# GATB/bcalm

Measured on AMD Instinct MI355X. Metric: distinct k-mers/s reads->unitigs k=31, higher is better.
Workload: dtype u64; 1 GPU; BASELINE config 3: synthetic 100000000 x 150 bp reads per GPU, k=31, abundance-min 2, 1% substitutions, 30x coverage; multi_gpu=single GPU, minimizer_size=16, log2_partitions=22

## Files before the change

bcalm_amd/csrc/host_ctx.h:

```cpp
#pragma once

namespace {

thread_local std::string g_err;
int fail(int code, const char* fmt, ...) {
    char buf[512];
    va_list ap; va_start(ap, fmt); vsnprintf(buf, sizeof buf, fmt, ap); va_end(ap);
    g_err = buf;
    return code;
}
#define HIPCK(call)                                                                                   \
    do {                                                                                              \
        hipError_t e_ = (call);                                                                       \
        if (e_ != hipSuccess)                                                                         \
            return fail(e_ == hipErrorOutOfMemory ? CDBG_E_NOMEM : CDBG_E_NODEVICE, "%s failed: %s (%s:%d)", \
                        #call, hipGetErrorString(e_), __FILE__, __LINE__);                            \
    } while (0)
#define CK(expr) do { int rc_ = (expr); if (rc_ != CDBG_OK) return rc_; } while (0)

struct DevPool {
    static constexpr size_t MIN_BYTES = 1u << 20;
    struct Block { void* p; size_t bytes; };
    std::mutex mu; std::vector<Block> blocks[64]; size_t held[64] = {}; size_t limit_[64] = {};
    static int device() { int d = 0; if (hipGetDevice(&d) != hipSuccess || d < 0 || d >= 64) d = 0; return d; }
// ... 230 lines not shown
    std::vector<uint64_t> run_off, run_start, run_place; std::vector<uint32_t> run_len; bool runs_ready = false;
    DBuf<uint32_t> comp, comp_first; DBuf<uint64_t> comp_unitigs, comp_bases, comp_kmers, comp_kc; bool comp_ready = false; uint64_t comp_info[5] = { 0, 0, 0, 0, 0 };
    DBuf<uint32_t> color_planes, color_ustart; uint32_t color_n = 0; uint64_t color_words = 0; bool color_opened = false; DBuf<uint64_t> color_out;
    DBuf<uint64_t> cl_run_off, cl_runs, cl_kmers; DBuf<uint32_t> cl_offset, cl_len, cl_cls, cl_ncol, cl_bits; bool cl_ready = false; uint64_t color_info[4] = { 0, 0, 0, 0 };
    DBuf<uint64_t> cq_seg_off, cq_seg_start, cq_seg_place; DBuf<uint32_t> cq_seg_len, cq_seg_cls, cq_found, cq_ncol, cq_bits;
    bool cq_ready = false; uint64_t cq_n = 0, cq_segs = 0;
    DBuf<uint4> rank_a, rank_b; DBuf<uint32_t> rank_flag;
    DBuf<uint4> walk_rec; DBuf<uint32_t> walk_heads, walk_hlen; DBuf<uint64_t> walk_hoff; bool walk_off = false;
    cdbg_transport tr{}; bool have_tr = false; uint64_t comm_bytes = 0;
    bool tr_ordered = false;
    bool force_multi = false;
#ifndef CDBG_HOSTSIM
    RcclComm* rccl = nullptr;
#endif
    DBuf<uint32_t> xcnt; DBuf<uint64_t> xoff, xbase, xrecs;
    uint64_t piece_lo = 0, piece_hi = 0;
    bool xchg_done = false;
    DBuf<uint8_t> xg[5], xsend;
    DBuf<uint8_t> dg_dest, dg_dense, dg_packed, dg_rpacked, dg_rdense; DBuf<uint64_t> dg_pos, dg_cnt, dg_wire_s, dg_wire_r, dg_meta_s, dg_meta_r, dg_boff, dg_uoff, dg_rboff, dg_rkc, dg_aoff, dg_raoff;
    DBuf<uint2> dg_pairs, dg_pair_s, dg_pair_r, dg_rs, dg_rr; DBuf<uint32_t> dg_qs, dg_qsrc, dg_qr, dg_lens, dg_alen, dg_rn, dg_rlens, dg_ab_s, dg_ab_r, dg_rab; DBuf<uint4> dg_rst;
};

namespace {

int stream_scan_dispatch(cdbg_ctx* c);
int ingest_init(cdbg_ctx* c) {
    if (c->pin[0]) return CDBG_OK;
    if (const char* e = c->knobs.get("CDBG_STAGE_BYTES")) c->stage_bytes = std::min<uint64_t>(cdbg_ctx::STAGE_BYTES, std::max<uint64_t>(64, strtoull(e, nullptr, 10)));
    HIPCK(hipStreamCreate(&c->copy_stream));
    for (int i = 0; i < 2; ++i) {
        if (hipHostMalloc((void**)&c->pin[i], cdbg_ctx::STAGE_BYTES) != hipSuccess) return fail(CDBG_E_NOMEM, "pinned staging buffer (%llu bytes)", (unsigned long long)cdbg_ctx::STAGE_BYTES);
        HIPCK(hipEventCreate(&c->pin_ev[i]));
    }
    return CDBG_OK;
}
void ingest_release(cdbg_ctx* c) {
    for (int i = 0; i < 2; ++i) {
        if (c->pin[i]) { (void)hipHostFree(c->pin[i]); (void)hipEventDestroy(c->pin_ev[i]); c->pin[i] = nullptr; }
    }
    for (auto& sg : c->stages) if (sg.p) { (void)hipHostFree(sg.p); (void)hipEventDestroy(sg.ev); }
    c->stages.clear();
    if (c->copy_stream) { (void)hipStreamDestroy(c->copy_stream); c->copy_stream = hipStream_t{}; }
}
int ingest_reserve(cdbg_ctx* c, uint64_t need) {
    while (c->prewarm_reads.load(std::memory_order_acquire)) std::this_thread::sleep_for(std::chrono::microseconds(200));
    if (c->reads.p && c->reads.cap >= need) return CDBG_OK;
    uint64_t cap = std::max<uint64_t>(c->reads.cap * 2, 256ull << 20);
    if (c->expect_bytes) cap = std::max<uint64_t>(cap, c->expect_bytes + c->expect_bytes / 64 + (8ull << 20));
    while (cap < need) cap *= 2;
    if (c->ss_on) HIPCK(hipStreamSynchronize(c->stream));
    DBuf<uint8_t> bigger;
    CK(bigger.alloc(cap, false));
    HIPCK(hipStreamSynchronize(c->copy_stream));
    if (c->n_dev) HIPCK(hipMemcpy(bigger.p, c->reads.p, c->n_dev, hipMemcpyDeviceToDevice));
    c->reads.swap(bigger);
    return CDBG_OK;
}
int ingest_flush(cdbg_ctx* c) {
    if (!c->pin_fill) return CDBG_OK;
    CK(ingest_reserve(c, c->n_dev + c->pin_fill));
    const int b = c->pin_cur;
    HIPCK(hipMemcpyAsync(c->reads.p + c->n_dev, c->pin[b], c->pin_fill, hipMemcpyHostToDevice, c->copy_stream));
    HIPCK(hipEventRecord(c->pin_ev[b], c->copy_stream));
    c->pin_busy[b] = true;
    c->n_dev += c->pin_fill; c->pin_fill = 0;
    c->pin_cur = b ^ 1;
    if (c->pin_busy[b ^ 1]) { HIPCK(hipEventSynchronize(c->pin_ev[b ^ 1])); c->pin_busy[b ^ 1] = false; }
    if (c->expect_bytes && c->prm.world_size == 1 && !c->force_multi) CK(stream_scan_dispatch(c));
    return CDBG_OK;
}
int ingest_append(cdbg_ctx* c, const char* src, uint64_t n) {
    CK(ingest_init(c));
    while (n) {
        const uint64_t room = c->stage_bytes - c->pin_fill, take = std::min(room, n);
        memcpy(c->pin[c->pin_cur] + c->pin_fill, src, take);
        c->pin_fill += take; src += take; n -= take;
        if (c->pin_fill == c->stage_bytes) CK(ingest_flush(c));
    }
    return CDBG_OK;
}
int stage_acquire(cdbg_ctx* c, char** buf, uint64_t* cap) {
    CK(ingest_init(c));
    for (;;) {
        int oldest = -1;
        for (int i = 0; i < (int)c->stages.size(); ++i) {
            cdbg_ctx::Stage& sg = c->stages[i];
            if (sg.state == 2 && hipEventQuery(sg.ev) == hipSuccess) sg.state = 0;
            if (sg.state == 0) { sg.state = 1; *buf = (char*)sg.p; *cap = c->stage_bytes; return CDBG_OK; }
            if (sg.state == 2 && oldest < 0) oldest = i;
        }
        if ((int)c->stages.size() >= 32 && oldest >= 0) { HIPCK(hipEventSynchronize(c->stages[oldest].ev)); continue; }
        if ((int)c->stages.size() < cdbg_ctx::MAX_STAGES) {
            cdbg_ctx::Stage sg;
            if (hipHostMalloc((void**)&sg.p, cdbg_ctx::STAGE_BYTES) != hipSuccess) return fail(CDBG_E_NOMEM, "pinned staging buffer (%llu bytes)", (unsigned long long)cdbg_ctx::STAGE_BYTES);
            if (hipEventCreate(&sg.ev) != hipSuccess) { (void)hipHostFree(sg.p); return fail(CDBG_E_NODEVICE, "hipEventCreate failed (staging buffer)"); }
            sg.state = 1; c->stages.push_back(sg);
            *buf = (char*)sg.p; *cap = c->stage_bytes; return CDBG_OK;
        }
        if (oldest < 0) return fail(CDBG_E_STATE, "cdbg_stage_acquire: all %d staging buffers are held by the caller", cdbg_ctx::MAX_STAGES);
        HIPCK(hipEventSynchronize(c->stages[oldest].ev));
    }
}
int ingest_flush(cdbg_ctx* c);
int stage_commit(cdbg_ctx* c, char* buf, uint64_t n) {
    cdbg_ctx::Stage* sg = nullptr;
    for (auto& x : c->stages) if ((char*)x.p == buf) sg = &x;
    if (!sg || sg->state != 1) return fail(CDBG_E_PARAM, "cdbg_stage_commit: not a buffer handed out by cdbg_stage_acquire");
    if (n > c->stage_bytes) return fail(CDBG_E_PARAM, "cdbg_stage_commit: %llu bytes in a buffer of %llu", (unsigned long long)n, (unsigned long long)c->stage_bytes);
    if (n && base_valid((uint8_t)buf[n - 1])) {
        if (n == c->stage_bytes) return fail(CDBG_E_PARAM, "cdbg_stage_commit: a full buffer must end with a separator");
        buf[n++] = '\n';
    }
    if (!n) { sg->state = 0; return CDBG_OK; }
    CK(ingest_flush(c));
    CK(ingest_reserve(c, c->n_dev + n));
    HIPCK(hipMemcpyAsync(c->reads.p + c->n_dev, buf, n, hipMemcpyHostToDevice, c->copy_stream));
    HIPCK(hipEventRecord(sg->ev, c->copy_stream));
    sg->state = 2;
    c->n_dev += n;
    if (c->expect_bytes && c->prm.world_size == 1 && !c->force_multi) CK(stream_scan_dispatch(c));
    return CDBG_OK;
}
int upload_pending(cdbg_ctx* c) {
    if (c->reads_final) return CDBG_OK;
    if (c->n_dev == 0 && c->pin_fill == 0) {
        if (c->prm.world_size > 1 || c->force_multi) {
            CK(c->reads.alloc(512, false));
            HIPCK(hipMemset(c->reads.p, '\n', 512));
            c->nbytes = 0; c->nbytes_padded = 256; c->reads_final = true;
        }
        return CDBG_OK;
    }
    CK(ingest_flush(c));
    const uint64_t n = c->n_dev;
    const uint64_t np = ((n + 15) / 16) * 16 + 256;
    CK(ingest_reserve(c, np));
    HIPCK(hipStreamSynchronize(c->copy_stream));
    HIPCK(hipMemset(c->reads.p + n, '\n', np - n));
    c->nbytes = n; c->nbytes_padded = np; c->reads_final = true;
    ingest_release(c);
    return CDBG_OK;
}

int read_u64(const uint64_t* dptr, uint64_t* out, size_t n = 1) {
    HIPCK(hipMemcpy(out, dptr, n * sizeof(uint64_t), hipMemcpyDeviceToHost));
    return CDBG_OK;
}
int read_u32(const uint32_t* dptr, uint32_t* out, size_t n = 1) {
    HIPCK(hipMemcpy(out, dptr, n * sizeof(uint32_t), hipMemcpyDeviceToHost));
    return CDBG_OK;
}
int check_device_error(cdbg_ctx* c, const char* where) {
    uint32_t e = 0; CK(read_u32(c->derr.p, &e));
    if (e) return fail(CDBG_E_INTERNAL, "%s: device reported error %u (1 solid overflow, 2 scratch sizing, 3 piece overflow, 4 unitig overflow, 5 glue log overflow, 9 junction-ownership flag of a k-mer wrong [simulator build only])", where, e);
    HIPCK(hipGetLastError());
    return CDBG_OK;
}
struct HostMarks {
    bool on = enabled(); double t0 = now();
    static bool enabled() { static const bool e = getenv("CDBG_HOST_MARKS") != nullptr; return e; }
    static double now() { timespec ts; clock_gettime(CLOCK_MONOTONIC, &ts); return ts.tv_sec * 1e3 + ts.tv_nsec * 1e-6; }
    void mark(const char* what) { if (!on) return; (void)hipDeviceSynchronize(); const double t = now(); fprintf(stderr, "[host] %-28s %8.2f ms\n", what, t - t0); t0 = t; }
};
struct Timer {
    hipEvent_t a{}, b{}; hipStream_t s{};
    int start(hipStream_t st) { s = st; HIPCK(hipEventCreate(&a)); HIPCK(hipEventCreate(&b)); HIPCK(hipEventRecord(a, s)); return CDBG_OK; }
    int stop(float* ms) { HIPCK(hipEventRecord(b, s)); HIPCK(hipEventSynchronize(b)); HIPCK(hipEventElapsedTime(ms, a, b)); (void)hipEventDestroy(a); (void)hipEventDestroy(b); return CDBG_OK; }
};

void configure(cdbg_ctx* c, uint64_t total_bytes) {
    const int W = c->W;
    const int ts = W == 1 ? TS_COUNT_1 : W == 2 ? TS_COUNT_2 : TS_COUNT_4;
#ifndef CDBG_OCC_NUM
#define CDBG_OCC_NUM 3
#define CDBG_OCC_DEN 2
#endif
    const bool sifted = W >= 3 && c->prm.abundance_min >= 2;
    const uint64_t target_occ = W >= 3 ? (uint64_t)ts * (sifted ? 12 : 6) / 10 : (uint64_t)ts * CDBG_OCC_NUM / CDBG_OCC_DEN;
    int log_np = c->log_np_override >= 0 ? c->log_np_override : c->prm.log2_partitions;
    if (log_np < 0) {
        log_np = 0;
        while (log_np < 24 && ((uint64_t)1 << log_np) * target_occ < total_bytes) ++log_np;
    }
    if (log_np < c->rank_bits) log_np = c->rank_bits;
    if (log_np > 26) log_np = 26;
    int m = c->prm.minimizer_size;
    if (m <= 0) m = std::min(16, std::max(6, (log_np + 10) / 2 + 1));
    m = std::max(1, std::min(m, std::min(16, c->k - 1)));
    c->log_np = log_np; c->m = m;
    c->n_local_parts = ((uint64_t)1 << log_np) >> c->rank_bits;
    c->st.minimizer_size = m; c->st.log2_partitions = log_np; c->st.kmer_words = W;
}

int exscan_u32(cdbg_ctx* c, const uint32_t* counts, uint64_t* off, uint64_t n) {
    hipStream_t s = c->stream;
    const uint64_t nb = (n + EXSCAN_BLOCK - 1) / EXSCAN_BLOCK;
    CK(c->exscan_tmp.alloc(nb + 1, false));
    if (n == 0) { HIPCK(hipMemsetAsync(off, 0, sizeof(uint64_t), s)); return CDBG_OK; }
    CDBG_LAUNCH(k_exscan_sums, nb, EXSCAN_THREADS, s, counts, c->exscan_tmp.p, n);
    CDBG_LAUNCH(k_exscan_top, 1, EXSCAN_THREADS, s, c->exscan_tmp.p, nb, off + n);
    CDBG_LAUNCH(k_exscan_apply, nb, EXSCAN_THREADS, s, counts, (const uint64_t*)c->exscan_tmp.p, off, n);
    return CDBG_OK;
}

int agree(cdbg_ctx* c, int rc, const char* where) {
    if (!(c->prm.world_size > 1 || c->force_multi) || !c->have_tr) return rc;
    const std::string mine = rc != CDBG_OK ? g_err : std::string();
    std::vector<uint64_t> all(c->prm.world_size); const uint64_t st = (uint64_t)(int64_t)rc;
    if (c->tr.all_gather_u64(c->tr.user, &st, all.data(), 1) != 0) return fail(CDBG_E_INTERNAL, "transport all_gather_u64 failed (%s)", where);
    if (rc != CDBG_OK) { g_err = mine; return rc; }
    for (int r = 0; r < c->prm.world_size; ++r)
        if (all[r] != 0) return fail(CDBG_E_INTERNAL, "%s: rank %d reported error %lld; all ranks stop", where, r, (long long)(int64_t)all[r]);
    return CDBG_OK;
}


}
```

bcalm_amd/csrc/host_glue.h:

```cpp
#pragma once

namespace {

template <int W>
int glue_join_impl(cdbg_ctx* c, bool sharded) {
    if (c->stage < 2) return fail(CDBG_E_STATE, "cdbg_glue before cdbg_compact");
    hipStream_t s = c->stream;
    const uint64_t NP = c->n_pieces;
    if (2 * NP >= 0x7FFFFFF0ULL) return fail(CDBG_E_INTERNAL, "too many pieces for 31-bit end ids (%llu)", (unsigned long long)NP);
    const uint32_t NS = (uint32_t)(2 * NP);
    Timer t; CK(t.start(s));
    CK(c->link.alloc(NS, false));
    HIPCK(hipMemsetAsync(c->link.p, 0xFF, (size_t)std::max<uint32_t>(NS, 1) * sizeof(uint32_t), s));
    HIPCK(hipMemsetAsync(c->dstats.p, 0, 32 * sizeof(uint64_t), s));
    HIPCK(hipMemsetAsync(c->derr.p, 0, 4 * sizeof(uint32_t), s));
    const uint32_t world = sharded ? (uint32_t)c->prm.world_size : 1u;
    const uint64_t n_mine = c->n_glog / world + (world > 1 ? (c->n_glog >> 6) + 1024 : 0);
    bool bucketed = (c->knobs.get("CDBG_GLUE_TABLE") == nullptr || c->direct_join) && c->n_glog > 0;
    if (bucketed && c->direct_join) {
        const uint64_t JB = 1ull << c->join_log_jb;
        JoinBucketParams bp{ c->jfill.p, c->jrecs.p, (uint32_t)JB, c->link.p, c->dstats.p, nullptr, nullptr, 0, nullptr };
        CDBG_LAUNCH((k_join_bucket<W>), std::min<uint64_t>((JB + 3) / 4, 256 * 16), JB_THREADS, s, bp);
    } else if (bucketed) {
        int log_jb = 0; while (((uint64_t)(JB_CAP / 2) << log_jb) < n_mine && log_jb < 26) ++log_jb;
        const uint64_t JB = 1ull << log_jb;
        CK(c->jfill.alloc(JB, false)); CK(c->jrecs.alloc(JB * JB_CAP * (W + 1), false));
        HIPCK(hipMemsetAsync(c->jfill.p, 0, JB * sizeof(uint32_t), s));
        JoinScatterParams sp{ c->glog_keys.p, c->glog_tag.p, c->n_glog, log_jb, c->jfill.p, c->jrecs.p, c->derr.p,
                              world - 1, world > 1 ? (uint32_t)c->prm.rank : 0u };
        CDBG_LAUNCH((k_join_scatter<W>), std::min<uint64_t>((c->n_glog + GLUE_THREADS - 1) / GLUE_THREADS, 1u << 16), GLUE_THREADS, s, sp);
        JoinBucketParams bp{ c->jfill.p, c->jrecs.p, (uint32_t)JB, c->link.p, c->dstats.p, nullptr, nullptr, 0, nullptr };
        CDBG_LAUNCH((k_join_bucket<W>), std::min<uint64_t>((JB + 3) / 4, 256 * 16), JB_THREADS, s, bp);
        HIPCK(hipStreamSynchronize(s));
        uint32_t e = 0; CK(read_u32(c->derr.p, &e));
        if (e == 8) {
            bucketed = false;
            HIPCK(hipMemsetAsync(c->link.p, 0xFF, (size_t)std::max<uint32_t>(NS, 1) * sizeof(uint32_t), s));
            HIPCK(hipMemsetAsync(c->dstats.p, 0, 32 * sizeof(uint64_t), s));
            HIPCK(hipMemsetAsync(c->derr.p, 0, 4 * sizeof(uint32_t), s));
        }
    }
    if (!bucketed && c->n_glog) {
        CK(glue_table_slots(n_mine + n_mine / 4 + 1024, &c->glue_cap));
        CK(c->glue_keys.alloc((uint64_t)c->glue_cap * W, false));
        CK(c->glue_a.alloc(c->glue_cap, false)); CK(c->glue_b.alloc(c->glue_cap, false)); CK(c->glue_conf.alloc(c->glue_cap, false));
        HIPCK(hipMemsetAsync(c->glue_keys.p, 0xFF, (uint64_t)c->glue_cap * W * sizeof(uint64_t), s));
        HIPCK(hipMemsetAsync(c->glue_a.p, 0, (uint64_t)c->glue_cap * sizeof(uint32_t), s));
        HIPCK(hipMemsetAsync(c->glue_b.p, 0, (uint64_t)c->glue_cap * sizeof(uint32_t), s));
        HIPCK(hipMemsetAsync(c->glue_conf.p, 0, (uint64_t)c->glue_cap * sizeof(uint32_t), s));
        GlueBuildParams bp{ c->glog_keys.p, c->glog_tag.p, c->n_glog, c->glue_keys.p, c->glue_a.p, c->glue_b.p, c->glue_conf.p, c->glue_cap - 1,
                            world - 1, world > 1 ? (uint32_t)c->prm.rank : 0u };
        CDBG_LAUNCH((k_glue_build<W>), std::min<uint64_t>((c->n_glog + GLUE_THREADS - 1) / GLUE_THREADS, MAX_GRID), GLUE_THREADS, s, bp);
        GlueResolveParams gp{};
        gp.keys = c->glue_keys.p; gp.a = c->glue_a.p; gp.b = c->glue_b.p; gp.conf = c->glue_conf.p;
        gp.cap = c->glue_cap; gp.W = W; gp.link = c->link.p; gp.stats = c->dstats.p;
        CDBG_LAUNCH(k_glue_resolve, std::min<uint64_t>((c->glue_cap + GLUE_THREADS - 1) / GLUE_THREADS, GLUE_RESOLVE_GRID), GLUE_THREADS, s, gp);
    }
    float ms = 0; CK(t.stop(&ms));
    CK(check_device_error(c, "glue join"));
    uint64_t gs = 0; CK(read_u64(c->dstats.p, &gs));
    c->n_join_local = gs; c->st.ms_glue = ms; c->joined = true;
    return CDBG_OK;
}


int glue_walk(cdbg_ctx* c, bool* done) {
    hipStream_t s = c->stream;
    const uint64_t NP = c->n_pieces, NS = 2 * NP;
    *done = false;
    if (!NP) return CDBG_OK;
    const uint64_t ucap = std::max<uint64_t>(NP, 1);
    const uint64_t ocap = std::max<uint64_t>(c->n_piece_bases, 1);
    CK(c->unitig_off.alloc(ucap, false)); CK(c->unitig_len.alloc(ucap, false)); CK(c->unitig_kc.alloc(ucap, false));
    CK(c->unitig_bases.alloc(ocap + 64, false));
    if (c->prm.all_abundance_counts) CK(c->unitig_ab.alloc(ocap, false));
    CK(c->rank_flag.alloc(4, true));
    CK(c->walk_rec.alloc(NS, false)); CK(c->walk_heads.alloc(NS, false)); CK(c->walk_hlen.alloc(NS, false)); CK(c->walk_hoff.alloc(NS, false));
    HIPCK(hipMemsetAsync(c->cursors.p + 2, 0, 2 * sizeof(uint64_t), s));
    HIPCK(hipMemsetAsync(c->dstats.p, 0, 32 * sizeof(uint64_t), s));
    HIPCK(hipMemsetAsync(c->derr.p, 0, 4 * sizeof(uint32_t), s));
    HIPCK(hipMemsetAsync(c->rank_flag.p, 0, sizeof(uint32_t), s));
    uint32_t max_steps = 4096;
    if (const char* e = c->knobs.get("CDBG_WALK_MAX")) max_steps = (uint32_t)strtoul(e, nullptr, 10);
    uint64_t* const n_heads = c->dstats.p + 6;
    WalkInitParams ip{ (uint32_t)NP, c->piece_n.p, c->piece_kc.p, c->piece_boff.p, c->link.p, c->walk_rec.p, c->walk_heads.p, n_heads, c->dstats.p + 4 };
    CDBG_LAUNCH(k_walk_init, (NP + WALK_PIECES - 1) / WALK_PIECES, WALK_THREADS, s, ip);
    const uint64_t spans = (NS + WALK_SPAN - 1) / WALK_SPAN, wave_grid = (spans + WALK_THREADS / 64 - 1) / (WALK_THREADS / 64);
    WalkMeasureParams mp{ c->walk_rec.p, c->walk_heads.p, n_heads, c->walk_hlen.p, max_steps, c->rank_flag.p };
    CDBG_LAUNCH(k_walk_measure, wave_grid, WALK_THREADS, s, mp);
    WalkPlaceParams pp{ n_heads, c->walk_hlen.p, c->walk_hoff.p, c->k, c->cursors.p + 2, c->cursors.p + 3, ucap, ocap, c->derr.p };
    CDBG_LAUNCH(k_walk_place, spans, WALK_THREADS, s, pp);
    WalkCopyParams wp{};
    wp.k = c->k; wp.rec = c->walk_rec.p; wp.piece_bases = c->piece_bases.p;
    wp.heads = c->walk_heads.p; wp.n_heads = n_heads; wp.hlen = c->walk_hlen.p; wp.hoff = c->walk_hoff.p;
    wp.unitig_off = c->unitig_off.p; wp.unitig_len = c->unitig_len.p; wp.unitig_kc = c->unitig_kc.p; wp.out = c->unitig_bases.p; wp.visited = c->dstats.p + 5;
    wp.piece_ab = c->prm.all_abundance_counts ? c->piece_ab.p : nullptr; wp.unitig_ab = c->unitig_ab.p;
    CDBG_LAUNCH(k_walk_copy, wave_grid, WALK_THREADS, s, wp);
    HIPCK(hipStreamSynchronize(s));
    uint64_t d[2]; CK(read_u64(c->dstats.p + 4, d, 2));
    uint32_t gave_up = 0; CK(read_u32(c->rank_flag.p, &gave_up));
    if (gave_up || d[1] != d[0]) { c->walk_off = true; return CDBG_OK; }
    *done = true;
    return CDBG_OK;
}

template <int W>
int glue_impl(cdbg_ctx* c) {
    if (c->stage < 2) return fail(CDBG_E_STATE, "cdbg_glue before cdbg_compact");
    if ((c->prm.world_size > 1 || c->force_multi) && c->have_tr && !c->xchg_done && !c->joined) {
        if (!c->prm.emit_replicated && c->knobs.get("CDBG_GLUE_REPLICATED") == nullptr) {
            const int rc = glue_sharded<W>(c);
            if (rc != DG_FALLBACK) return rc;
        }
        CK(glue_exchange(c));
    }
    if (!c->joined) CK(glue_join_impl<W>(c, false));
    hipStream_t s = c->stream;
    const uint64_t NP = c->n_pieces;
    const uint32_t NS = (uint32_t)(2 * NP);
    const float ms_join = c->st.ms_glue;
    HostMarks hm;
    Timer t; CK(t.start(s));
    bool walked = false;
    if (c->prm.world_size <= 1 && !c->force_multi && !c->xchg_done && !c->walk_off && c->knobs.get("CDBG_GLUE_RANK") == nullptr) CK(glue_walk(c, &walked));
    if (walked) {
        { uint64_t cur[2]; CK(read_u64(c->cursors.p + 2, cur, 2)); c->n_unitigs = cur[0]; c->unitig_total = cur[1]; }
        CK(pack_unitigs(c));
        float ms_fin = 0; CK(t.stop(&ms_fin));
        hm.mark("glue: walk + copy");
        c->st.ms_glue = ms_join + ms_fin;
        CK(check_device_error(c, "glue"));
        c->joined = false;
        c->st.n_glue_joined = c->n_join_local; c->st.n_unitigs = c->n_unitigs; c->st.unitig_bases = c->unitig_total; c->st.n_walked_unitigs = c->n_unitigs;
        c->st.ms_total += c->st.ms_glue;
        c->stage = 3;
        return CDBG_OK;
    }
    DBuf<uint32_t>& flag = c->rank_flag; DBuf<uint4>& st_a = c->rank_a; DBuf<uint4>& st_b = c->rank_b;
    CK(st_a.alloc(NS, false)); CK(st_b.alloc(NS, false));
    CK(flag.alloc(4, true));
    HIPCK(hipMemsetAsync(c->dstats.p, 0, 32 * sizeof(uint64_t), s));
    HIPCK(hipMemsetAsync(c->derr.p, 0, 4 * sizeof(uint32_t), s));
    uint32_t* const link_p = c->link.p;

    uint64_t n_cycles_cut = 0;
    const uint32_t gridS = (NS + GLUE_THREADS - 1) / GLUE_THREADS;
    RankParams rp{};
    uint4* fa_st = nullptr;
    const uint2* st8 = nullptr; uint4* hinfo = nullptr;
    bool ranked = false;
    if (NS) {
        int max_rounds8 = 2; while ((1ull << (max_rounds8 - 1)) < NS) ++max_rounds8;
        Rank8Params r8{ NS, link_p, c->piece_n.p, reinterpret_cast<uint2*>(st_b.p), flag.p };
        CDBG_LAUNCH(k_rank8_init, gridS, GLUE_THREADS, s, r8);
        for (int r = 0; r < max_rounds8 && !ranked; ++r) {
            HIPCK(hipMemsetAsync(flag.p, 0, sizeof(uint32_t), s));
            CDBG_LAUNCH(k_rank8_jump, gridS, GLUE_THREADS, s, r8);
            HIPCK(hipStreamSynchronize(s));
            uint32_t ch = 0; CK(read_u32(flag.p, &ch));
            if (!ch) ranked = true;
        }
        if (ranked) { st8 = r8.a; hinfo = st_a.p; }
    }
    if (NS && !ranked) {
        int max_rounds = 2; while ((1ull << (max_rounds - 1)) < NS) ++max_rounds;
        for (int pass = 0; pass < 2; ++pass) {
            rp.n_states = NS; rp.link = link_p; rp.piece_n = c->piece_n.p;
            rp.st_a = st_a.p; rp.st_b = st_b.p; rp.changed = flag.p;
            CDBG_LAUNCH(k_rank_init, gridS, GLUE_THREADS, s, rp);
            bool converged = false;
            for (int r = 0; r < max_rounds; ++r) {
                HIPCK(hipMemsetAsync(flag.p, 0, sizeof(uint32_t), s));
                CDBG_LAUNCH(k_rank_jump, gridS, GLUE_THREADS, s, rp);
                std::swap(rp.st_a, rp.st_b);
                HIPCK(hipStreamSynchronize(s));
                uint32_t ch = 0; CK(read_u32(flag.p, &ch));
                if (!ch) { converged = true; break; }
            }
            fa_st = rp.st_a;
            if (converged) break;
            if (pass == 1) return fail(CDBG_E_INTERNAL, "list ranking did not converge after cutting cycles");
            HIPCK(hipMemsetAsync(flag.p, 0, sizeof(uint32_t), s));
            CutParams cu{ NS, rp.st_a, link_p, flag.p };
            CDBG_LAUNCH(k_cut_cycles, gridS, GLUE_THREADS, s, cu);
            HIPCK(hipStreamSynchronize(s));
            uint32_t nc = 0; CK(read_u32(flag.p, &nc)); n_cycles_cut += nc;
        }
    }
    if (NS && !st8) {
        uint4* const other = (fa_st == st_a.p) ? st_b.p : st_a.p;
        RankNarrowParams np{ NS, fa_st, reinterpret_cast<uint2*>(other) };
        CDBG_LAUNCH(k_rank_narrow, gridS, GLUE_THREADS, s, np);
        st8 = reinterpret_cast<const uint2*>(other); hinfo = fa_st;
    }
    const uint64_t ucap = std::max<uint64_t>(NP, 1);
    const uint64_t ocap = std::max<uint64_t>(c->n_piece_bases, 1);
    CK(c->unitig_off.alloc(ucap, false)); CK(c->unitig_len.alloc(ucap, false)); CK(c->unitig_kc.alloc(ucap, false));
    CK(c->unitig_bases.alloc(ocap + 64, false));
    if (c->prm.all_abundance_counts) CK(c->unitig_ab.alloc(ocap, false));
    HIPCK(hipMemsetAsync(c->cursors.p + 2, 0, 2 * sizeof(uint64_t), s));
    if (NS) {
        HeadParams hp{};
        hp.n_states = NS; hp.k = c->k; hp.link = link_p; hp.st = st8; hp.hinfo = hinfo;
        hp.unitig_off = c->unitig_off.p; hp.unitig_len = c->unitig_len.p; hp.unitig_kc = c->unitig_kc.p;
        hp.unitig_cap = ucap; hp.out_cap = ocap; hp.n_unitigs = c->cursors.p + 2; hp.out_cursor = c->cursors.p + 3; hp.error = c->derr.p;
        hp.own_lo = 0; hp.own_hi = NS;
        if (c->prm.world_size > 1 && !c->prm.emit_replicated && c->xchg_done) { hp.own_lo = (uint32_t)(2 * c->piece_lo); hp.own_hi = (uint32_t)(2 * c->piece_hi); }
        CDBG_LAUNCH(k_unitig_heads, (NS + HEADS_PER_WG - 1) / HEADS_PER_WG, GLUE_THREADS, s, hp);
        EmitParams ep{};
        ep.n_pieces = (uint32_t)NP; ep.k = c->k; ep.st = st8; ep.hinfo = hp.hinfo;
        ep.piece_n = c->piece_n.p; ep.piece_kc = c->piece_kc.p; ep.piece_boff = c->piece_boff.p; ep.piece_bases = c->piece_bases.p;
        ep.unitig_kc = c->unitig_kc.p; ep.out = c->unitig_bases.p;
        ep.piece_ab = c->prm.all_abundance_counts ? c->piece_ab.p : nullptr; ep.unitig_ab = c->unitig_ab.p;
        CDBG_LAUNCH(k_emit, (uint32_t)((NP + GLUE_THREADS - 1) / GLUE_THREADS), GLUE_THREADS, s, ep);
    }
    { uint64_t cur[2]; CK(read_u64(c->cursors.p + 2, cur, 2)); c->n_unitigs = cur[0]; c->unitig_total = cur[1]; }
    CK(pack_unitigs(c));
    float ms_fin = 0; CK(t.stop(&ms_fin));
    hm.mark("glue: rank + heads + emit");
    c->st.ms_glue = ms_join + ms_fin;
    CK(check_device_error(c, "glue"));
    c->joined = false;
    c->st.n_glue_joined = c->n_join_local; c->st.n_unitigs = c->n_unitigs; c->st.unitig_bases = c->unitig_total; c->st.n_cycles += n_cycles_cut;
    c->st.ms_total += c->st.ms_glue;
    c->stage = 3;
    return CDBG_OK;
}

struct UnitigView { uint64_t U; const uint64_t* off; const uint32_t* len; const uint8_t* bases; uint64_t total_bases; };

template <int W>
int links_build(cdbg_ctx* c, const UnitigView& v, DBuf<uint64_t>& link_off, DBuf<uint32_t>& link_to, uint64_t& n_links) {
    hipStream_t s = c->stream;
    const uint64_t U = v.U, NE = 2 * U;
    if (pow2_at_least(4 * U + 64) > (1ull << 30)) return fail(CDBG_E_INTERNAL, "too many unitigs (%llu) for the 30-bit slots of the link table", (unsigned long long)U);
    const uint32_t cap = (uint32_t)pow2_at_least(4 * U + 64);
    DBuf<uint64_t> lk_keys; DBuf<uint32_t> lk_cnt, lk_ends, end_slot, deg;
    CK(lk_keys.alloc((uint64_t)cap * W, false)); CK(lk_cnt.alloc((uint64_t)cap * 2, true));
    CK(lk_ends.alloc((uint64_t)cap * 2 * LINK_PER_FLAG, false)); CK(end_slot.alloc(NE, false)); CK(deg.alloc(NE, false));
    HIPCK(hipMemsetAsync(lk_keys.p, 0xFF, (uint64_t)cap * W * sizeof(uint64_t), s));
    CK(link_off.alloc(NE + 1, true));
    LinkParams lp{};
    lp.n_unitigs = U; lp.k = c->k; lp.unitig_off = v.off; lp.unitig_len = v.len; lp.bases = v.bases;
    lp.lk_keys = lk_keys.p; lp.lk_cnt = lk_cnt.p; lp.lk_ends = lk_ends.p; lp.lk_mask = cap - 1;
    lp.end_slot = end_slot.p; lp.deg = deg.p;
    n_links = 0;
    if (NE) {
        const uint64_t grid = (NE + LINK_THREADS - 1) / LINK_THREADS;
        CDBG_LAUNCH((k_link_insert<W>), grid, LINK_THREADS, s, lp);
        CDBG_LAUNCH(k_link_count, grid, LINK_THREADS, s, lp);
// ... 163 lines not shown
```

bcalm_amd/csrc/k_walk.h:

```cpp
#pragma once
#include "k_glue.h"

namespace cdbg {

constexpr int WALK_THREADS = 256;
constexpr int WALK_PPT = 8;
constexpr int WALK_PIECES = WALK_THREADS * WALK_PPT;
constexpr int WALK_SPAN = 1024;
constexpr int WALK_SPT = WALK_SPAN / WALK_THREADS;

struct WalkInitParams { uint32_t n_pieces; const uint32_t* piece_n; const uint64_t* piece_kc; const uint64_t* piece_boff; const uint32_t* link;
                        uint4* rec; uint32_t* heads; uint64_t* n_heads; uint64_t* n_live; };
__global__ void __launch_bounds__(WALK_THREADS) k_walk_init(WalkInitParams P) {
    CDBG_SHARED uint32_t s_wn[WALK_THREADS / 64], s_wl[WALK_THREADS / 64]; CDBG_SHARED uint64_t s_base;
    const int tid = threadIdx.x, lane = tid & 63, wave = tid >> 6;
    const uint32_t p0 = blockIdx.x * (uint32_t)WALK_PIECES + (uint32_t)wave * (64u * WALK_PPT) + (uint32_t)lane;
    uint32_t hs[2 * WALK_PPT], at[WALK_PPT]; uint32_t run = 0, live = 0;
#pragma unroll
    for (int i = 0; i < WALK_PPT; ++i) {
        const uint32_t p = p0 + 64u * (uint32_t)i;
        hs[2 * i] = NONE32; hs[2 * i + 1] = NONE32;
        uint32_t cnt = 0;
        if (p < P.n_pieces) {
            const uint32_t n = P.piece_n[p];
            uint4 a, b; a.x = NONE32; a.y = NONE32; a.z = n; a.w = 0; b.x = 0; b.y = 0; b.z = 0; b.w = 0;
            if (n) {
                const uint64_t kc = P.piece_kc[p], bo = P.piece_boff[p];
                const uint2 l = reinterpret_cast<const uint2*>(P.link)[p];
                a.x = l.y; a.y = l.x;
                a.w = (uint32_t)kc; b.x = (uint32_t)(kc >> 32); b.y = (uint32_t)bo; b.z = (uint32_t)(bo >> 32);
                ++live;
                if (l.x == NONE32) { hs[2 * i] = 2 * p; ++cnt; }
                if (l.y == NONE32) { hs[2 * i + 1] = 2 * p + 1; ++cnt; }
            }
            P.rec[2 * (uint64_t)p] = a; P.rec[2 * (uint64_t)p + 1] = b;
        }
        const uint32_t incl = wave_incl_sum_u32(cnt);
        at[i] = run + incl - cnt;
        run += wave_readlane_u32(incl, 63);
    }
    const uint32_t lsum = wave_readlane_u32(wave_incl_sum_u32(live), 63);
    if (lane == 0) { s_wn[wave] = run; s_wl[wave] = lsum; }
    __syncthreads();
    uint32_t wbase = 0, tot = 0, ltot = 0;
    for (int w = 0; w < WALK_THREADS / 64; ++w) { if (w < wave) wbase += s_wn[w]; tot += s_wn[w]; ltot += s_wl[w]; }
    if (tid == 0) {
        s_base = tot ? atomic_add_u64(P.n_heads, (uint64_t)tot) : 0ull;
        if (ltot) atomic_add_u64(P.n_live, (uint64_t)ltot);
    }
    __syncthreads();
    uint32_t* const out = P.heads + s_base + wbase;
#pragma unroll
    for (int i = 0; i < WALK_PPT; ++i) {
        uint32_t j = at[i];
        if (hs[2 * i] != NONE32) out[j++] = hs[2 * i];
        if (hs[2 * i + 1] != NONE32) out[j] = hs[2 * i + 1];
    }
}

CDBG_DEV void walk_copy(const uint8_t* src, uint8_t* dst, uint32_t nb, uint32_t skip, bool fwd) {
    uint32_t i = skip;
    if (nb - skip >= 8u) {
        for (;;) {
            if (i + 8u > nb) { if (i == nb) break; i = nb - 8u; }
            const uint64_t w = fwd ? ld_unaligned_u64(src + i) : comp_ascii8_rev(ld_unaligned_u64(src + (nb - 8u - i)));
            st_unaligned_u64(dst + i, w);
            i += 8u;
        }
    } else {
        uint64_t w = 0; const uint32_t r = nb - skip;
        for (uint32_t j = 0; j < r; ++j) w |= (uint64_t)(fwd ? src[skip + j] : comp_ascii(src[nb - 1 - skip - j])) << (8 * j);
        if (r & 4u) { st_unaligned_u32(dst + i, (uint32_t)w); w >>= 32; i += 4u; }
        if (r & 2u) { st_unaligned_u16(dst + i, (uint16_t)w); w >>= 16; i += 2u; }
        if (r & 1u) dst[i] = (uint8_t)w;
    }
}

CDBG_DEV uint32_t walk_lane_rank(uint64_t mask, int lane) { return (uint32_t)__popcll(mask & ((1ULL << lane) - 1ULL)); }

struct WalkMeasureParams { const uint4* rec; const uint32_t* heads; const uint64_t* n_heads; uint32_t* hlen; uint32_t max_steps; uint32_t* giveup; };
__global__ void __launch_bounds__(WALK_THREADS) k_walk_measure(WalkMeasureParams P) {
    const int lane = threadIdx.x & 63;
    const uint64_t n_heads = *P.n_heads;
    const uint64_t wv = ((uint64_t)blockIdx.x * WALK_THREADS + threadIdx.x) >> 6;
    uint64_t next = wv * WALK_SPAN; const uint64_t end = next + WALK_SPAN < n_heads ? next + WALK_SPAN : n_heads;
    bool active = false; uint32_t e = 0, h = 0, len = 0, steps = 0; uint64_t idx = 0;
    for (;;) {
        const uint64_t need = __ballot(!active);
        if (next < end) {
            const uint64_t my = next + walk_lane_rank(need, lane);
            if (!active && my < end) { idx = my; h = P.heads[my]; e = h; len = 0; steps = 0; active = true; }
            next += (uint64_t)__popcll(need);
        }
        if (!__any(active)) break;
        if (active) {
            const uint4 a = P.rec[2 * (uint64_t)(e >> 1)];
            len += a.z;
            const uint32_t nx = (e & 1u) ? a.y : a.x;
            if (nx == NONE32) { P.hlen[idx] = e > (h ^ 1u) ? len : 0u; active = false; }
            else if (++steps > P.max_steps) { *P.giveup = 1u; P.hlen[idx] = 0u; active = false; }
            else e = nx;
        }
    }
}

struct WalkPlaceParams { const uint64_t* n_heads; uint32_t* hlen; uint64_t* hoff; int k; uint64_t* n_unitigs; uint64_t* out_cursor; uint64_t unitig_cap, out_cap; uint32_t* error; };
__global__ void __launch_bounds__(WALK_THREADS) k_walk_place(WalkPlaceParams P) {
    CDBG_SHARED uint32_t s_wn[WALK_THREADS / 64]; CDBG_SHARED uint64_t s_wl[WALK_THREADS / 64];
    CDBG_SHARED uint64_t s_ubase, s_obase;
    const int tid = threadIdx.x, lane = tid & 63, wave = tid >> 6;
    const uint64_t n_heads = *P.n_heads;
    if ((uint64_t)blockIdx.x * WALK_SPAN >= n_heads) return;
    const uint64_t i0 = (uint64_t)blockIdx.x * WALK_SPAN + (uint64_t)tid * WALK_SPT;
    uint32_t kl[WALK_SPT]; uint32_t kn = 0; uint64_t ksum = 0;
#pragma unroll
    for (int i = 0; i < WALK_SPT; ++i) {
        kl[i] = i0 + i < n_heads ? P.hlen[i0 + i] : 0u;
        if (kl[i]) { ++kn; ksum += (uint64_t)kl[i] + (uint64_t)P.k - 1u; }
    }
    uint32_t icnt = kn; uint64_t isum = ksum;
#pragma unroll
    for (int d = 1; d < 64; d <<= 1) {
        const uint32_t c = __shfl_up(icnt, (unsigned)d); const uint64_t l = __shfl_up(isum, (unsigned)d);
        if (lane >= d) { icnt += c; isum += l; }
    }
    if (lane == 63) { s_wn[wave] = icnt; s_wl[wave] = isum; }
    __syncthreads();
    uint32_t my_i = icnt - kn, tot_n = 0; uint64_t my_o = isum - ksum, tot_l = 0;
    for (int w = 0; w < WALK_THREADS / 64; ++w) {
        if (w < wave) { my_i += s_wn[w]; my_o += s_wl[w]; }
        tot_n += s_wn[w]; tot_l += s_wl[w];
    }
    if (tid == 0 && tot_n) {
        s_ubase = atomic_add_u64(P.n_unitigs, (uint64_t)tot_n);
        s_obase = atomic_add_u64(P.out_cursor, tot_l);
        if (s_ubase + tot_n > P.unitig_cap || s_obase + tot_l > P.out_cap) *P.error = 4;
    }
    __syncthreads();
    if (!tot_n) return;
    const bool fits = s_ubase + tot_n <= P.unitig_cap && s_obase + tot_l <= P.out_cap;
    uint64_t uid = s_ubase + my_i, off = s_obase + my_o;
#pragma unroll
    for (int i = 0; i < WALK_SPT; ++i) {
        if (!kl[i]) continue;
        P.hlen[i0 + i] = fits ? (uint32_t)uid + 1u : 0u; P.hoff[i0 + i] = off;
        ++uid; off += (uint64_t)kl[i] + (uint64_t)P.k - 1u;
    }
}

struct WalkCopyParams {
    int k; const uint4* rec; const uint8_t* piece_bases;
    const uint32_t* heads; const uint64_t* n_heads; const uint32_t* hlen; const uint64_t* hoff;
    uint64_t* unitig_off; uint32_t* unitig_len; uint64_t* unitig_kc; uint8_t* out; uint64_t* visited;
    const uint32_t* piece_ab; uint32_t* unitig_ab;
};
__global__ void __launch_bounds__(WALK_THREADS) k_walk_copy(WalkCopyParams P) {
    const int lane = threadIdx.x & 63;
    const uint64_t n_heads = *P.n_heads;
    const uint64_t wv = ((uint64_t)blockIdx.x * WALK_THREADS + threadIdx.x) >> 6;
    uint64_t next = wv * WALK_SPAN; const uint64_t end = next + WALK_SPAN < n_heads ? next + WALK_SPAN : n_heads;
    bool active = false; uint32_t e = 0, koff = 0, uid = 0, seen = 0; uint64_t kc = 0, uoff = 0;
    for (;;) {
        const uint64_t need = __ballot(!active);
        if (next < end) {
            const uint64_t my = next + walk_lane_rank(need, lane);
            if (!active && my < end) {
                const uint32_t u1 = P.hlen[my];
                if (u1) { uid = u1 - 1u; uoff = P.hoff[my]; e = P.heads[my]; koff = 0; kc = 0; active = true; }
            }
            next += (uint64_t)__popcll(need);
        }
        if (!__any(active)) { if (next < end) continue; break; }
        if (active) {
            const uint32_t p = e >> 1;
            const uint4 a = P.rec[2 * (uint64_t)p], b = P.rec[2 * (uint64_t)p + 1];
            const uint32_t n = a.z, nb = n + (uint32_t)P.k - 1u;
            const uint64_t boff = (uint64_t)b.y | ((uint64_t)b.z << 32);
            kc += (uint64_t)a.w | ((uint64_t)b.x << 32);
            const bool fwd = (e & 1u) == END_LEFT;
            walk_copy(P.piece_bases + boff, P.out + uoff + koff, nb, koff ? (uint32_t)P.k - 1u : 0u, fwd);
            if (P.piece_ab) {
                const uint32_t* sa = P.piece_ab + boff + (P.k - 1);
                uint32_t* da = P.unitig_ab + uoff + koff + (P.k - 1);
                if (fwd) { for (uint32_t t = 0; t < n; ++t) da[t] = sa[t]; }
                else { for (uint32_t t = 0; t < n; ++t) da[t] = sa[n - 1 - t]; }
            }
            koff += n; ++seen;
            const uint32_t nx = (e & 1u) ? a.y : a.x;
            if (nx == NONE32) { P.unitig_off[uid] = uoff; P.unitig_len[uid] = koff + (uint32_t)P.k - 1u; P.unitig_kc[uid] = kc; active = false; }
            else e = nx;
        }
    }
    const uint64_t s64 = wave_sum_u64((uint64_t)seen);
    if (lane == 0 && s64) atomic_add_u64(P.visited, s64);
}

}
```

Baseline: 24.97 billion kmers/s.

## Coalesce unitig base writes into aligned 16-byte stores in walk copy

Replaces the per-piece walk_copy in k_walk_copy with a per-lane sliding 16-byte window. Bases are read in 8-byte chunks, reverse-complemented when needed, and written as aligned 16-byte stores, with special handling for the unaligned head and tail of each unitig. Writing unitig_off and unitig_len moves into k_walk_place, so the copy kernel no longer stores them. The goal is fewer, wider, aligned global writes, in exchange for more complex boundary logic and extra register state per lane.

```diff
diff --git a/bcalm_amd/csrc/host_ctx.h b/bcalm_amd/csrc/host_ctx.h
--- a/bcalm_amd/csrc/host_ctx.h
+++ b/bcalm_amd/csrc/host_ctx.h
@@ -406,7 +406,7 @@
 }
 int check_device_error(cdbg_ctx* c, const char* where) {
     uint32_t e = 0; CK(read_u32(c->derr.p, &e));
-    if (e) return fail(CDBG_E_INTERNAL, "%s: device reported error %u (1 solid overflow, 2 scratch sizing, 3 piece overflow, 4 unitig overflow, 5 glue log overflow, 9 junction-ownership flag of a k-mer wrong [simulator build only])", where, e);
+    if (e) return fail(CDBG_E_INTERNAL, "%s: device reported error %u (1 solid overflow, 2 scratch sizing, 3 piece overflow, 4 unitig overflow, 5 glue log overflow, 9 junction-ownership flag of a k-mer wrong [simulator build only], 10 k_walk_copy stored outside its lane's unitig [simulator build only])", where, e);
     HIPCK(hipGetLastError());
     return CDBG_OK;
 }
diff --git a/bcalm_amd/csrc/host_glue.h b/bcalm_amd/csrc/host_glue.h
--- a/bcalm_amd/csrc/host_glue.h
+++ b/bcalm_amd/csrc/host_glue.h
@@ -88,14 +88,16 @@
     const uint64_t spans = (NS + WALK_SPAN - 1) / WALK_SPAN, wave_grid = (spans + WALK_THREADS / 64 - 1) / (WALK_THREADS / 64);
     WalkMeasureParams mp{ c->walk_rec.p, c->walk_heads.p, n_heads, c->walk_hlen.p, max_steps, c->rank_flag.p };
     CDBG_LAUNCH(k_walk_measure, wave_grid, WALK_THREADS, s, mp);
-    WalkPlaceParams pp{ n_heads, c->walk_hlen.p, c->walk_hoff.p, c->k, c->cursors.p + 2, c->cursors.p + 3, ucap, ocap, c->derr.p };
+    WalkPlaceParams pp{ n_heads, c->walk_hlen.p, c->walk_hoff.p, c->k, c->cursors.p + 2, c->cursors.p + 3, ucap, ocap, c->derr.p,
+                        c->unitig_off.p, c->unitig_len.p };
     CDBG_LAUNCH(k_walk_place, spans, WALK_THREADS, s, pp);
     WalkCopyParams wp{};
     wp.k = c->k; wp.rec = c->walk_rec.p; wp.piece_bases = c->piece_bases.p;
     wp.heads = c->walk_heads.p; wp.n_heads = n_heads; wp.hlen = c->walk_hlen.p; wp.hoff = c->walk_hoff.p;
-    wp.unitig_off = c->unitig_off.p; wp.unitig_len = c->unitig_len.p; wp.unitig_kc = c->unitig_kc.p; wp.out = c->unitig_bases.p; wp.visited = c->dstats.p + 5;
-    wp.piece_ab = c->prm.all_abundance_counts ? c->piece_ab.p : nullptr; wp.unitig_ab = c->unitig_ab.p;
-    CDBG_LAUNCH(k_walk_copy, wave_grid, WALK_THREADS, s, wp);
+    wp.unitig_len = c->unitig_len.p; wp.unitig_kc = c->unitig_kc.p; wp.out = c->unitig_bases.p; wp.visited = c->dstats.p + 5;
+    wp.piece_ab = c->prm.all_abundance_counts ? c->piece_ab.p : nullptr; wp.unitig_ab = c->unitig_ab.p; wp.error = c->derr.p;
+    if (c->k >= 9) CDBG_LAUNCH(k_walk_copy<true>, wave_grid, WALK_THREADS, s, wp);
+    else CDBG_LAUNCH(k_walk_copy<false>, wave_grid, WALK_THREADS, s, wp);
     HIPCK(hipStreamSynchronize(s));
     uint64_t d[2]; CK(read_u64(c->dstats.p + 4, d, 2));
     uint32_t gave_up = 0; CK(read_u32(c->rank_flag.p, &gave_up));
diff --git a/bcalm_amd/csrc/k_walk.h b/bcalm_amd/csrc/k_walk.h
--- a/bcalm_amd/csrc/k_walk.h
+++ b/bcalm_amd/csrc/k_walk.h
@@ -104,7 +104,8 @@
     }
 }
 
-struct WalkPlaceParams { const uint64_t* n_heads; uint32_t* hlen; uint64_t* hoff; int k; uint64_t* n_unitigs; uint64_t* out_cursor; uint64_t unitig_cap, out_cap; uint32_t* error; };
+struct WalkPlaceParams { const uint64_t* n_heads; uint32_t* hlen; uint64_t* hoff; int k; uint64_t* n_unitigs; uint64_t* out_cursor; uint64_t unitig_cap, out_cap; uint32_t* error;
+                         uint64_t* unitig_off; uint32_t* unitig_len; };
 __global__ void __launch_bounds__(WALK_THREADS) k_walk_place(WalkPlaceParams P) {
     CDBG_SHARED uint32_t s_wn[WALK_THREADS / 64]; CDBG_SHARED uint64_t s_wl[WALK_THREADS / 64];
     CDBG_SHARED uint64_t s_ubase, s_obase;
@@ -143,30 +144,102 @@
 #pragma unroll
     for (int i = 0; i < WALK_SPT; ++i) {
         if (!kl[i]) continue;
+        const uint32_t len = kl[i] + (uint32_t)P.k - 1u;
         P.hlen[i0 + i] = fits ? (uint32_t)uid + 1u : 0u; P.hoff[i0 + i] = off;
-        ++uid; off += (uint64_t)kl[i] + (uint64_t)P.k - 1u;
+        if (fits) { P.unitig_off[uid] = off; P.unitig_len[uid] = len; }
+        ++uid; off += (uint64_t)len;
     }
 }
 
 struct WalkCopyParams {
     int k; const uint4* rec; const uint8_t* piece_bases;
     const uint32_t* heads; const uint64_t* n_heads; const uint32_t* hlen; const uint64_t* hoff;
-    uint64_t* unitig_off; uint32_t* unitig_len; uint64_t* unitig_kc; uint8_t* out; uint64_t* visited;
+    const uint32_t* unitig_len; uint64_t* unitig_kc; uint8_t* out; uint64_t* visited;
     const uint32_t* piece_ab; uint32_t* unitig_ab;
+    uint32_t* error;
 };
+
+struct WalkWin { uint64_t lo, hi, prev; uint32_t st; };
+struct WalkDst { uint8_t* out; uint64_t u0; uint32_t ulen; uint32_t* error; uint32_t flushes; };
+
+CDBG_DEV void wc_guard(WalkDst& D, uint64_t at, uint32_t bytes) {
+#ifdef CDBG_HOSTSIM
+    if (at < D.u0 || at + bytes > D.u0 + D.ulen) *D.error = 10;
+#endif
+}
+CDBG_DEV void wc_st16(WalkDst& D, uint64_t at, uint64_t lo, uint64_t hi) {
+    wc_guard(D, at, 16);
+#ifdef CDBG_HOSTSIM
+    if (at & 15u) *D.error = 10;
+    __builtin_memcpy(D.out + at, &lo, 8); __builtin_memcpy(D.out + at + 8, &hi, 8);
+#else
+    uint4 v; v.x = (uint32_t)lo; v.y = (uint32_t)(lo >> 32); v.z = (uint32_t)hi; v.w = (uint32_t)(hi >> 32);
+    *reinterpret_cast<uint4*>(D.out + at) = v;
+#endif
+}
+CDBG_DEV void wc_st8(WalkDst& D, uint64_t at, uint64_t w) { wc_guard(D, at, 8); st_unaligned_u64(D.out + at, w); }
+CDBG_DEV uint64_t wc_bytes8(uint64_t a, uint64_t b, uint32_t r) { return r == 0u ? a : r == 8u ? b : (a >> (8u * r)) | (b << (64u - 8u * r)); }
+CDBG_DEV void wc_store_small(WalkDst& D, uint64_t at, uint64_t w0, uint64_t w1, uint64_t w2, uint32_t n) {
+    wc_st8(D, at, w0);
+    if (n >= 16u) { wc_st8(D, at + 8u, w1); if (n > 16u) wc_st8(D, at + n - 8u, wc_bytes8(w1, w2, n - 16u)); }
+    else wc_st8(D, at + n - 8u, wc_bytes8(w0, w1, n - 8u));
+}
+CDBG_DEV void wc_flush(WalkWin& B, WalkDst& D, uint64_t cb) {
+    ++D.flushes;
+    if (cb >= D.u0) {
+        wc_st16(D, cb, B.lo, B.hi);
+        if (B.st == 1u) { const uint32_t h = 16u - ((uint32_t)D.u0 & 15u); wc_st8(D, D.u0, B.prev | (B.lo << (8u * h))); }
+        B.prev = B.hi; B.st = 2u;
+    } else {
+        const uint32_t a = (uint32_t)(D.u0 - cb);
+        if (a <= 8u) { wc_st8(D, D.u0, wc_bytes8(B.lo, B.hi, a)); if (a < 8u) wc_st8(D, cb + 8u, B.hi); B.prev = B.hi; B.st = 2u; }
+        else { B.prev = B.hi >> (8u * (a - 8u)); B.st = 1u; }
+    }
+}
+CDBG_DEV void wc_append(WalkWin& B, WalkDst& D, uint64_t pos, uint64_t w, uint32_t c) {
+    const uint32_t s = (uint32_t)pos & 15u;
+    if (s < 8u) { B.lo |= w << (8u * s); if (s) B.hi |= w >> (64u - 8u * s); }
+    else {
+        const uint32_t s8 = s - 8u;
+        B.hi |= w << (8u * s8);
+        if (s + c >= 16u) { wc_flush(B, D, pos - s); B.lo = s8 ? w >> (64u - 8u * s8) : 0ull; B.hi = 0; }
+    }
+}
+CDBG_DEV void wc_finish(WalkWin& B, WalkDst& D, uint64_t end) {
+    const uint32_t t = (uint32_t)end & 15u;
+    if (B.st == 2u) {
+        if (t >= 8u) { wc_st8(D, end - t, B.lo); if (t > 8u) wc_st8(D, end - 8u, wc_bytes8(B.lo, B.hi, t - 8u)); }
+        else if (t) wc_st8(D, end - 8u, wc_bytes8(B.prev, B.lo, t));
+    } else if (B.st == 1u) {
+        const uint32_t h = 16u - ((uint32_t)D.u0 & 15u);
+        wc_store_small(D, D.u0, B.prev | (B.lo << (8u * h)), (B.lo >> (64u - 8u * h)) | (B.hi << (8u * h)), B.hi >> (64u - 8u * h), h + t);
+    } else {
+        const uint32_t a = (uint32_t)D.u0 & 15u;
+        wc_store_small(D, D.u0, wc_bytes8(B.lo, B.hi, a), B.hi >> (8u * a), 0, (uint32_t)(end - D.u0));
+    }
+}
+
+template <bool CHUNKED>
 __global__ void __launch_bounds__(WALK_THREADS) k_walk_copy(WalkCopyParams P) {
     const int lane = threadIdx.x & 63;
     const uint64_t n_heads = *P.n_heads;
     const uint64_t wv = ((uint64_t)blockIdx.x * WALK_THREADS + threadIdx.x) >> 6;
     uint64_t next = wv * WALK_SPAN; const uint64_t end = next + WALK_SPAN < n_heads ? next + WALK_SPAN : n_heads;
     bool active = false; uint32_t e = 0, koff = 0, uid = 0, seen = 0; uint64_t kc = 0, uoff = 0;
+    WalkWin B{ 0, 0, 0, 0 }; WalkDst D{ P.out, 0, 0, P.error, 0 };
     for (;;) {
         const uint64_t need = __ballot(!active);
         if (next < end) {
             const uint64_t my = next + walk_lane_rank(need, lane);
             if (!active && my < end) {
                 const uint32_t u1 = P.hlen[my];
-                if (u1) { uid = u1 - 1u; uoff = P.hoff[my]; e = P.heads[my]; koff = 0; kc = 0; active = true; }
+                if (u1) {
+                    uid = u1 - 1u; uoff = P.hoff[my]; e = P.heads[my]; koff = 0; kc = 0; active = true;
+                    B.lo = 0; B.hi = 0; B.st = 0; D.u0 = uoff;
+#ifdef CDBG_HOSTSIM
+                    D.ulen = P.unitig_len[uid];
+#endif
+                }
             }
             next += (uint64_t)__popcll(need);
         }
@@ -178,7 +251,30 @@
             const uint64_t boff = (uint64_t)b.y | ((uint64_t)b.z << 32);
             kc += (uint64_t)a.w | ((uint64_t)b.x << 32);
             const bool fwd = (e & 1u) == END_LEFT;
-            walk_copy(P.piece_bases + boff, P.out + uoff + koff, nb, koff ? (uint32_t)P.k - 1u : 0u, fwd);
+            const uint32_t skip = koff ? (uint32_t)P.k - 1u : 0u;
+            if constexpr (CHUNKED) {
+                const uint8_t* const src = P.piece_bases + boff;
+                uint64_t pos = uoff + koff + skip;
+                D.flushes = 0;
+                for (uint32_t i = skip; i < nb;) {
+                    const uint32_t c = nb - i < 8u ? nb - i : 8u, j = i + c - 8u;
+                    const uint64_t w = fwd ? ld_unaligned_u64(src + j) : comp_ascii8_rev(ld_unaligned_u64(src + (nb - 8u - j)));
+                    wc_append(B, D, pos, w >> (8u * (8u - c)), c);
+                    pos += c; i += c;
+                }
+#ifdef CDBG_HOSTSIM
+                if (const char* tf = getenv("CDBG_SIM_WALK_TRACE")) if (FILE* fp = fopen(tf, "a")) {
+                    fprintf(fp, "%u %llu %u %u %d %u %d\n", uid, (unsigned long long)uoff, koff + skip, nb - skip, fwd ? 1 : 0, D.flushes,
+                            ((e & 1u) ? a.y : a.x) == NONE32 ? 1 : 0);
+                    fclose(fp);
+                }
+#endif
+            } else {
+#ifdef CDBG_HOSTSIM
+                wc_guard(D, uoff + koff + skip, nb - skip);
+#endif
+                walk_copy(P.piece_bases + boff, P.out + uoff + koff, nb, skip, fwd);
+            }
             if (P.piece_ab) {
                 const uint32_t* sa = P.piece_ab + boff + (P.k - 1);
                 uint32_t* da = P.unitig_ab + uoff + koff + (P.k - 1);
@@ -187,7 +283,10 @@
             }
             koff += n; ++seen;
             const uint32_t nx = (e & 1u) ? a.y : a.x;
-            if (nx == NONE32) { P.unitig_off[uid] = uoff; P.unitig_len[uid] = koff + (uint32_t)P.k - 1u; P.unitig_kc[uid] = kc; active = false; }
+            if (nx == NONE32) {
+                if constexpr (CHUNKED) wc_finish(B, D, uoff + koff + (uint32_t)P.k - 1u);
+                P.unitig_kc[uid] = kc; active = false;
+            }
             else e = nx;
         }
     }
```

Result: faster. 25.31 billion kmers/s, median of 6 (+1.4%).
